# COMBINE-lab/RapMap

Hardware: AMD Instinct MI355X
Metric: Mreads/s (paired 2x100 bp; one unit = one read pair) (higher is better)
Workload: dtype u8/int32/u64 (integer & byte work, no floating point)

## Files before the change

rapmap_amd/csrc/qm_device.h:

```cpp
#pragma once
#include <hip/hip_runtime.h>
#include <stddef.h>

#define QMK_BLOCKS_PER_CU 8
#define QM_SEL_CHUNKS_B 4
#define QMK_DEFAULT_WPS 8
#define QMK_WPS_PH 6
#define QMK_WPS_NIP 8
#define QMK_WPS_PHNIP 6

extern "C" {
hipError_t qmk_build_sainfo(const unsigned int* SA, long long nSA, const unsigned int* offsets, long long T, void* out, hipStream_t st);
hipError_t qmk_build_saext(const unsigned char* text, long long n, const unsigned int* SA, long long nSA, int k, const void* sainfo, void* out, hipStream_t st);
hipError_t qmk_build_saext2(const unsigned char* text, long long n, const unsigned int* SA, long long nSA, int k, const void* sainfo, void* out, hipStream_t st);
size_t qmk_saext2_bytes(void);
hipError_t qmk_build_sanext(const unsigned char* text, long long n, const unsigned int* SA, long long nSA, int k, unsigned int* out, hipStream_t st);
hipError_t qmk_build_slots(const void* recs, long long K, void* slots, unsigned long long cap, int k, hipStream_t st);
hipError_t qmk_build_slots_from_ph(const void* dev_index, long long n, void* slots, unsigned long long cap, unsigned long long* d_bad, hipStream_t st);
hipError_t qmk_build_phrecs(const unsigned int* data, const unsigned char* lens, long long n, const void* dev_index, void* out, hipStream_t st);
hipError_t qmk_build_phfilter(const void* recs, long long n, void* filter, unsigned long long mask, int k, hipStream_t st);
int qmk_map_grid(long long n, int num_cu);
int qmk_map_grid_ex(long long n, int num_cu, int ph_compact);
int qmk_grid_oversub_ph(void);
int qmk_grid_oversub(void);
int qmk_resident_grid(long long n, int num_cu);
hipError_t qmk_launch_reads_ns2(const void* dev_index, const void* read_batch, int collect, int grid, int num_cu, hipStream_t st);
hipError_t qmk_launch_reads_ns3(const void* dev_index, const void* read_batch, int collect, int grid, int num_cu, hipStream_t st);
hipError_t qmk_launch_reads_ns4(const void* dev_index, const void* read_batch, int collect, int grid, int num_cu, hipStream_t st);
hipError_t qmk_launch_reads_ns8(const void* dev_index, const void* read_batch, int collect, int grid, int num_cu, hipStream_t st);
hipError_t qmk_launch_reads_ns32(const void* dev_index, const void* read_batch, int collect, int grid, int num_cu, hipStream_t st);
hipError_t qmk_launch_lean(const void* dev_index, const void* read_batch, int num_cu, hipStream_t st);
hipError_t qmk_launch_lean_nq(const void* dev_index, const void* read_batch, int num_cu, hipStream_t st);
hipError_t qmk_launch_duo(const void* dev_index, const void* read_batch, int num_cu, hipStream_t st);
hipError_t qmk_map_reads(const void* dev_index, const void* read_batch, int ns, int grid, int num_cu, hipStream_t st);
hipError_t qmk_map_reads_ex(const void* dev_index, const void* read_batch, int ns, int collect, int grid, int num_cu, hipStream_t st);
hipError_t qmk_h2m(const void* dev_index, const void* read_batch, int grid, int num_cu, hipStream_t st);
hipError_t qmk_h2m_packw(const void* dev_index, const void* read_batch, const long long* ids, const unsigned long long* nids, long long* todoq, int grid, int num_cu, hipStream_t st);
hipError_t qmk_rebase_offsets(const long long* src, long long* dst, long long n, long long add, hipStream_t st);
hipError_t qmk_h2m_pack(const void* dev_index, const void* read_batch, long long* todoq, int grid, int num_cu, hipStream_t st);
hipError_t qmk_sel_merge(const void* pair_batch, const void* sel_batch, hipStream_t st);
size_t qmk_sel_scratch_bytes(void);
size_t qmk_sel_dyn_struct_bytes(void);
unsigned long long qmk_sel_dyn_bytes(long long n);
void qmk_sel_dyn_bind(void* host_struct, void* dev_base, long long n);
hipError_t qmk_collect_marked(const unsigned int* lcnt, long long nreads, unsigned int mark, long long* q, long long cap, unsigned long long* count, hipStream_t st);
hipError_t qmk_sel_slots(const void* pair_batch, hipStream_t st);
hipError_t qmk_sel_plan(const void* pair_batch, const void* sel_batch, int num_cu, hipStream_t st);
size_t qmk_sel_side_bytes(void);
hipError_t qmk_sel_align_finish(const void* pair_batch, const void* sel_batch, int num_cu, hipStream_t st);
size_t qmk_sel_task_bytes(void);
size_t qmk_sel_gmem_rows_bytes(int num_cu);
hipError_t qmk_sel_compact(const void* pair_batch, const void* tmp, const void* toff, hipStream_t st);
hipError_t qmk_pair_count(const void* pair_batch, hipStream_t st);
hipError_t qmk_pair_write(const void* pair_batch, hipStream_t st);
hipError_t qmk_unpack_reads(const unsigned char* packed, const long long* off, long long n, long long total_chars, unsigned char* seq,
                            const void* exc, long long n_exc, hipStream_t st);
size_t qmk_scan_temp_bytes(long long n);
hipError_t qmk_scan_counts(void* temp, size_t temp_bytes, const unsigned int* cnt, long long* offs, long long n,
                           hipStream_t st);
hipError_t qmk_scan_counts_masked(void* temp, size_t temp_bytes, const unsigned int* cnt, long long* offs, long long n, hipStream_t st);
hipError_t qmk_stage_gather(long long nreads, const unsigned int* ivcnt, const long long* ivoff, const void* iv, const long long* ivcsr, void* iv_out,
                            const unsigned int* lcnt, const long long* loff, const unsigned long long* lists, const long long* lcsr,
                            unsigned long long* words_out, hipStream_t st);
hipError_t qmk_eqc_label_queued(const void* src, long long nq, hipStream_t st);
hipError_t qmk_eqc_reset_probes(unsigned long long* q, long long n, hipStream_t st);
hipError_t qmk_eqc_sum(const unsigned long long* count, const unsigned long long* key, long long cap, unsigned long long* out, hipStream_t st);
int qmk_fld_grid(long long n_units, int num_cu, int max_blocks);
hipError_t qmk_fld_fold(const void* src, const void* acc, int blocks, hipStream_t st);
}
```

rapmap_amd/csrc/qm_host.hip:

```cpp
#include <fcntl.h>
#include <hip/hip_runtime.h>
#include <sys/mman.h>
#include <sys/stat.h>
#include <unistd.h>

#include <atomic>
#include <cmath>
#include <cstdarg>
#include <cstdio>
#include <cstdlib>
#include <cstring>
#include <deque>
#include <string>
#include <vector>
#include <thread>
#include <map>
#include <memory>
#include <mutex>
#include <condition_variable>
#include <functional>

#include "qm_mapper.inl"
#include "qm_lean.inl"
#include "qm_device.h"
// ... 176 lines not shown
  std::vector<std::thread> th; std::mutex mu; std::condition_variable cv, done;
  std::function<void(int)> job; unsigned long gen = 0; int pending = 0, parts = 0; bool stop = false;
  explicit SplitPool(int n) {
    for (int i = 0; i < n; ++i) th.emplace_back([this, i]() {
      unsigned long seen = 0;
      for (;;) {
        std::function<void(int)> j;
        { std::unique_lock<std::mutex> lk(mu); cv.wait(lk, [&] { return stop || (gen != seen && i < parts); }); if (stop) return; seen = gen; j = job; }
        j(i);
        { std::lock_guard<std::mutex> lk(mu); if (--pending == 0) done.notify_all(); }
      }
    });
  }
  void run(int n, std::function<void(int)> f) {
    std::unique_lock<std::mutex> lk(mu);
    job = std::move(f); parts = n; pending = n; ++gen;
    cv.notify_all();
    done.wait(lk, [&] { return pending == 0; });
  }
  ~SplitPool() { { std::lock_guard<std::mutex> lk(mu); stop = true; } cv.notify_all(); for (auto& t : th) t.join(); }
};
struct SplitJoin {
  qm_ctx* owner; int K; std::mutex mu; std::condition_variable cv;
  long long total[8] = {0}, base[9] = {0}; int arrived = 0; bool ready = false; int failed = 0;
  int arrive(int part, long long tot, long long& b, qm_hit*& dst);
  void abort(int rc) { std::lock_guard<std::mutex> lk(mu); if (!failed) failed = rc ? rc : QM_E_STATE; cv.notify_all(); }
  bool stagger = false; int turn = 0;
  int wait_turn(int part) {
    if (!stagger) return QM_OK;
    std::unique_lock<std::mutex> lk(mu);
    cv.wait(lk, [&] { return turn >= part || failed; });
    return failed ? fail(failed, "another part of the batch failed") : QM_OK;
  }
  void pass_turn(int part) { if (!stagger) return; std::lock_guard<std::mutex> lk(mu); if (turn < part + 1) turn = part + 1; cv.notify_all(); }
};

static void begin_call(qm_ctx* c) { c->last.invalidate(); c->stats = CallStats(); }

extern "C" {

const char* qm_last_error(void) { return g_err; }
const char* qm_version(void) { return "qmap_mi355 0.1 (RapMap 0.6.0 quasimap hot path, gfx950)"; }

int qm_opts_default(qm_opts* o) {
  if (!o) return fail(QM_E_ARG, "null opts");
  o->sensitive = 1; o->strict_check = 1; o->max_num_hits = 200; o->no_orphans = 0; o->no_dovetail = 0;
  o->fuzzy = 0; o->max_interval = 1000; o->sel_aln = 0; o->quasi_cov = 0.0;
  o->hard_filter = 0; o->match_score = 2; o->mismatch_penalty = -4; o->gap_open = 4; o->gap_extend = 2; o->dp_bandwidth = 15;
// ... 439 lines not shown

static int check_opts(const qm_opts* o) {
  if (!o) return fail(QM_E_ARG, "null opts");
  if (o->max_num_hits < 0 || o->max_interval < 1) return fail(QM_E_ARG, "bad max_num_hits / max_interval");
  return QM_OK;
}

struct ChunkFeeder {
  int64_t chunk;
  int (*upload)(void* self, int64_t u0, int64_t u1);
  void* self;
};

enum { QM_RUN_FUSED = 0, QM_RUN_COLLECT = 1, QM_RUN_FROM_INTERVALS = 2 };
struct RunReq {
  int mode = QM_RUN_FUSED;
  bool keepIntervals = false;
  bool keepFound = false;
  bool mergeOnly = false;
  bool stageView = false;
  bool longReads = false;
  int shortLen = 0;
  const qm_sa_interval_hit* ivIn = nullptr; const long long* ivInOff = nullptr; const int* lenIn = nullptr; const unsigned char* foundIn = nullptr;
  SplitJoin* join = nullptr; int part = 0;
  bool noDuo = false;
};

static DevIndex dev_index(const qm_ctx* c) {
  const Replica& R = *c->rep;
  DevIndex ix; ix.text = R.text; ix.n = c->ix->n; ix.SA = R.SA; ix.nSA = c->ix->nSA;
  ix.sainfo = (const SaInfo*)R.sainfo.p; ix.slots = (const Bucket*)R.slots.p; ix.hmask = R.cap - 1; ix.ph = R.ph; ix.k = c->ix->k;
  memset(&ix.phv, 0, sizeof(ix.phv)); if (R.ph) ix.phv = R.hPh;
  ix.sanext = c->d_sanext; ix.saext = (const SaExt*)R.saext.p; ix.saext2 = (const SaExt2*)c->d_saext2;
  return ix;
}


static bool ensure_saext2(qm_ctx* c) {
  if (c->d_saext2) return true;
  Replica& R = *c->rep;
  if (!R.saext || c->ix->nSA <= 0 || c->ix->nTxp >= (1LL << QM_EXT2_TID_BITS)) return false;
  std::lock_guard<std::mutex> lk(R.sanextMu);
  if (!R.saext2 && !R.saext2Tried) {
    R.saext2Tried = true;
    size_t freeB = 0, totalB = 0;
    const size_t need = (size_t)c->ix->nSA * qmk_saext2_bytes(), margin = (size_t)8 << 30;
    if (hipMemGetInfo(&freeB, &totalB) != hipSuccess || freeB < need + margin) { (void)hipGetLastError(); return false; }
// ... 349 lines not shown
  return c->d_scanTmp.ensure((int64_t)(stb ? stb : 16));
}

static int run_stage_b(qm_ctx* c, const qm_opts* o, const RunReq& rq, int64_t n, bool paired, const void* d_seq1, const void* d_off1,
                       const void* d_seq2, const void* d_off2, u64* hscal, long long& total) {
  int rc;
  if ((rc = c->d_cnt.ensure(n + 1))) return rc;
  if ((rc = c->d_offs.ensure(n + 1))) return rc;
  if ((rc = ensure_scan_tmp(c, n + 1))) return rc;
  PairBatch P; memset(&P, 0, sizeof(P));
  P.n = n; P.paired = paired ? 1 : 0; P.off1 = (const long long*)d_off1; P.off2 = (const long long*)d_off2;
  P.lcnt = c->d_lcnt; P.loff = c->d_loff; P.lists = c->d_lists; P.cnt = c->d_cnt; P.offs = c->d_offs;
  P.counters = c->d_scal + 1; P.max_num_hits = o->max_num_hits; P.no_orphans = rq.mergeOnly ? 0 : o->no_orphans;
  P.no_dovetail = rq.mergeOnly ? 0 : o->no_dovetail; P.fuzzy = o->fuzzy; P.merge_only = rq.mergeOnly ? 1 : 0;
  if (rq.mergeOnly) {
    if ((rc = c->d_tooMany.ensure(n + 1))) return rc;
    HIPCHK(hipMemsetAsync(c->d_tooMany, 0, (size_t)(n + 1), c->stream));
    P.too_many = c->d_tooMany;
  }
  if (rq.mergeOnly) c->last.tooManyUnits = n;
  HIPCHK(hipMemsetAsync(c->d_cnt + n, 0, sizeof(uint32_t), c->stream));
  if (o->sel_aln) {
    HIPCHK(qmk_sel_slots(&P, c->stream));
    HIPCHK(qmk_scan_counts(c->d_scanTmp, (size_t)c->d_scanTmp.cap, c->d_cnt, c->d_offs, n + 1, c->stream));
    if ((rc = c->d_toff.ensure(n + 1))) return rc;
    HIPCHK(hipMemcpyAsync(c->d_toff, c->d_offs, (size_t)(n + 1) * 8, hipMemcpyDeviceToDevice, c->stream));
    long long slots = 0;
    HIPCHK(hipMemcpyAsync(&slots, c->d_offs + n, sizeof(long long), hipMemcpyDeviceToHost, c->stream));
    const char* cuEnv = getenv("QM_SEL_CHUNK_UNITS");
    const int64_t minChunk = cuEnv && atoll(cuEnv) > 0 ? atoll(cuEnv) : 65536;
    const int K = n >= (int64_t)QM_SEL_CHUNKS_B * minChunk ? QM_SEL_CHUNKS_B : 1;
    long long cu[QM_SEL_CHUNKS_B + 1], cslot[QM_SEL_CHUNKS_B + 1];
    for (int i = 0; i <= K; ++i) { cu[i] = n * i / K; cslot[i] = 0; }
    for (int i = 1; i < K; ++i) HIPCHK(hipMemcpyAsync(&cslot[i], c->d_offs + cu[i], sizeof(long long), hipMemcpyDeviceToHost, c->stream));
    HIPCHK(hipStreamSynchronize(c->stream));
    cslot[K] = slots;
    if ((rc = c->d_tmp.ensure(slots + 1))) return rc;
    if ((rc = c->d_tsc.ensure(2 * slots + 2))) return rc;
    SelBatch A; memset(&A, 0, sizeof(A));
    A.seq1 = (const unsigned char*)d_seq1; A.seq2 = (const unsigned char*)d_seq2; A.text = c->rep->text;
    A.txp_off = c->rep->txpOff; A.txp_len = c->rep->txpLen; A.tmp = c->d_tmp; A.toff = c->d_toff; A.tsc = c->d_tsc;
    A.match = o->match_score; A.mismatch = o->mismatch_penalty; A.gap_open = o->gap_open; A.gap_extend = o->gap_extend;
    A.long_reads = rq.longReads ? 1 : 0;
    if (rq.longReads && !rq.mergeOnly && sel_ksw_ring_slots(o->dp_bandwidth) > 128) {
      if ((rc = c->d_kswRows.ensure((int64_t)qmk_sel_gmem_rows_bytes(c->numCU)))) return rc;
      A.ksw_rows = c->d_kswRows;
    }
// ... 15 lines not shown
      HIPCHK(hipStreamWaitEvent(c->planStream, c->evPlan[QM_SEL_CHUNKS_B], 0));
      SelBatch Ak[QM_SEL_CHUNKS_B];
      static const bool serial = [] { const char* e = getenv("QM_SEL_SERIAL"); return e && atoi(e) != 0; }();
      hipStream_t planStream = K > 1 && !serial ? c->planStream : c->stream;
      for (int i = 0; i < K; ++i) {
        Ak[i] = A; Ak[i].u0 = cu[i]; Ak[i].u1 = cu[i + 1];
        Ak[i].tasks = (SelTask*)(c->d_tasks + (size_t)(2 * cslot[i] + 2 * i) * qmk_sel_task_bytes());
        Ak[i].ntasks = c->d_ntk + i;
        Ak[i].sides = (SelSide*)(c->d_sides + (size_t)(2 * cslot[i] + 2 * i) * qmk_sel_side_bytes());
        Ak[i].nsides = c->d_ntk + QM_SEL_CHUNKS_B + i;
        Ak[i].torder = c->d_torder + (size_t)(2 * cslot[i] + 2 * i);
        if (!noStrip) { Ak[i].torder2 = c->d_torder + (size_t)(2 * slots + 2 * K + 2) + (size_t)(2 * cslot[i] + 2 * i); Ak[i].ntasks2 = c->d_ntk + 2 * QM_SEL_CHUNKS_B + i; }
        HIPCHK(qmk_sel_plan(&P, &Ak[i], c->numCU, planStream));
        if (K > 1) HIPCHK(hipEventRecord(c->evPlan[i], planStream));
      }
      for (int i = 0; i < K; ++i) {
        if (K > 1) HIPCHK(hipStreamWaitEvent(c->stream, c->evPlan[i], 0));
        HIPCHK(qmk_sel_align_finish(&P, &Ak[i], c->numCU, c->stream));
      }
    }
  } else {
    HIPCHK(qmk_pair_count(&P, c->stream));
  }
  HIPCHK(qmk_scan_counts(c->d_scanTmp, (size_t)c->d_scanTmp.cap, c->d_cnt, c->d_offs, n + 1, c->stream));
  total = 0;
  HIPCHK(hipMemcpyAsync(&total, c->d_offs + n, sizeof(long long), hipMemcpyDeviceToHost, c->stream));
  HIPCHK(hipMemcpyAsync(hscal, c->d_scal, QM_SC_WORDS * sizeof(u64), hipMemcpyDeviceToHost, c->stream));
  u64 h[3 * QM_SEL_CHUNKS_B];
  const bool selStats = o->sel_aln && !rq.mergeOnly;
  if (selStats) HIPCHK(hipMemcpyAsync(h, c->d_ntk, sizeof(h), hipMemcpyDeviceToHost, c->stream));
  HIPCHK(hipStreamSynchronize(c->stream));
  if (selStats) {
    for (int i = 0; i < QM_SEL_CHUNKS_B; ++i) { c->stats.kswTasks += (int64_t)h[i]; c->stats.selQuestions += (int64_t)h[QM_SEL_CHUNKS_B + i]; c->stats.stripTasks += (int64_t)h[2 * QM_SEL_CHUNKS_B + i]; }
    static const bool dbg = [] { const char* e = getenv("QM_SEL_DEBUG"); return e && atoi(e) != 0; }();
    if (dbg) fprintf(stderr, "[qm -s] %lld units: %lld alignment questions beyond PERFECT chains, %lld ksw2 alignments, %lld strip alignments\n", (long long)n, (long long)c->stats.selQuestions, (long long)c->stats.kswTasks, (long long)c->stats.stripTasks);
  }
  if (rq.join) {
    long long b = 0; qm_hit* dst = nullptr;
    if ((rc = rq.join->arrive(rq.part, total, b, dst))) return rc;
    P.hits = dst + b;
  } else {
    if ((rc = c->d_hits.ensure((int64_t)total + 1, total / 8))) return rc;
    P.hits = c->d_hits;
  }
  if (o->sel_aln) HIPCHK(qmk_sel_compact(&P, c->d_tmp, c->d_toff, c->stream));
  else HIPCHK(qmk_pair_write(&P, c->stream));
  return QM_OK;
}

static int map_device_impl(qm_ctx* c, const qm_opts* o, int64_t n, const void* d_seq1, const void* d_off1, const void* d_seq2,
                           const void* d_off2, int32_t max_read_len, int64_t* n_hits, qm_counters* counters, ChunkFeeder* feeder,
                           const RunReq& rq = RunReq(), int32_t short_read_len = 0) {
  if (!c || n < 0 || (n > 0 && (!d_seq1 || !d_off1))) return fail(QM_E_ARG, "bad argument");
  int rc = check_opts(o);
  if (rc) return rc;
  if ((d_seq2 == nullptr) != (d_off2 == nullptr)) return fail(QM_E_ARG, "seq2/off2 must both be given or both be null");
  HIPCHK(hipSetDevice(c->device));
  const int pick = (max_read_len > QM_MAX_READ_LEN && short_read_len > 0) ? short_read_len : (max_read_len > QM_MAX_READ_LEN ? QM_MAX_READ_LEN : max_read_len);
  const int ns = pick <= 128 ? 2 : (pick <= 192 ? 3 : (pick <= 256 ? 4 : 8));
  const bool paired = d_seq2 != nullptr;
  u64 hscal[QM_SC_WORDS];
  begin_call(c);
  HIPCHK(hipEventRecord(c->evA, c->stream));
  RunReq r2 = rq;
  r2.keepIntervals = rq.keepIntervals || c->debug != 0;
  r2.longReads = max_read_len > QM_MAX_READ_LEN;
  r2.shortLen = pick;
  if (rq.join && (rc = rq.join->wait_turn(rq.part))) return rc;
  rc = run_stage_a(c, o, r2, n, d_seq1, d_off1, d_seq2, d_off2, ns, feeder, hscal);
  if (rq.join) rq.join->pass_turn(rq.part);
  if (rc) return rc;
  if (r2.stageView) {
    const int64_t nreads = paired ? 2 * n : n;
    if ((rc = c->d_ivcsr.ensure(nreads + 1))) return rc;
    if ((rc = c->d_lcsr.ensure(nreads + 1))) return rc;
    if ((rc = c->h_tot.ensure(2))) return rc;
    if ((rc = ensure_scan_tmp(c, nreads + 1))) return rc;
    if (!r2.keepIntervals) {
      if ((rc = c->d_ivcnt.ensure(nreads + 1))) return rc;
      if ((rc = c->d_ivoff.ensure(nreads + 1))) return rc;
      if ((rc = c->d_iv.ensure(1))) return rc;
      HIPCHK(hipMemsetAsync(c->d_ivcnt, 0, (size_t)(nreads + 1) * sizeof(uint32_t), c->stream));
      HIPCHK(hipMemsetAsync(c->d_ivoff, 0, (size_t)(nreads + 1) * sizeof(long long), c->stream));
    }
    HIPCHK(hipMemsetAsync(c->d_ivcnt + nreads, 0, sizeof(uint32_t), c->stream));
    HIPCHK(hipMemsetAsync(c->d_lcnt + nreads, 0, sizeof(uint32_t), c->stream));
    HIPCHK(qmk_scan_counts(c->d_scanTmp, (size_t)c->d_scanTmp.cap, c->d_ivcnt, c->d_ivcsr, nreads + 1, c->stream));
    HIPCHK(qmk_scan_counts_masked(c->d_scanTmp, (size_t)c->d_scanTmp.cap, c->d_lcnt, c->d_lcsr, nreads + 1, c->stream));
    HIPCHK(hipMemcpyAsync(&c->h_tot[0], c->d_ivcsr + nreads, sizeof(long long), hipMemcpyDeviceToHost, c->stream));
    HIPCHK(hipMemcpyAsync(&c->h_tot[1], c->d_lcsr + nreads, sizeof(long long), hipMemcpyDeviceToHost, c->stream));
    c->last.stReads = nreads;
  }
  long long total = 0;
  if ((rc = run_stage_b(c, o, r2, n, paired, d_seq1, d_off1, d_seq2, d_off2, hscal, total))) return rc;
  HIPCHK(hipEventRecord(c->evB, c->stream));
  HIPCHK(hipStreamSynchronize(c->stream));
  float ms = 0; hipEventElapsedTime(&ms, c->evA, c->evB); c->last.totalMs = ms;
  c->last.units = n; c->last.hits = total; c->last.paired = paired;
  if (r2.stageView) c->last.stUnits = n;
  if (n_hits) *n_hits = total;
  if (counters) *counters = counters_from(hscal);
  return QM_OK;
}

int SplitJoin::arrive(int part, long long tot, long long& b, qm_hit*& dst) {
  std::unique_lock<std::mutex> lk(mu);
  total[part] = tot;
  if (++arrived == K && !failed) {
    for (int i = 0; i < K; ++i) base[i + 1] = base[i] + total[i];
    const int rc = owner->d_hits.ensure((int64_t)base[K] + 1, base[K] / 8);
    if (rc) failed = rc; else ready = true;
    cv.notify_all();
  }
  cv.wait(lk, [&] { return ready || failed; });
  if (failed) return failed == QM_E_NOMEM ? fail(QM_E_NOMEM, "hipMalloc of the result array failed") : fail(failed, "another part of the batch failed");
  b = base[part]; dst = owner->d_hits;
  return QM_OK;
}

static int map_device_split(qm_ctx* c, const qm_opts* o, int K, int64_t n, const void* d_seq1, const void* d_off1, const void* d_seq2,
                            const void* d_off2, int32_t max_read_len, int64_t* n_hits, qm_counters* counters) {
  int rc;
  HIPCHK(hipSetDevice(c->device));
  while ((int)c->helpers.size() < K) {
    qm_ctx* h = nullptr;
    if ((rc = qm_ctx_create_ex(c->ix, c->device, c->flags, &h))) return rc;
    h->isHelper = true; c->helpers.push_back(h);
  }
  if (!c->pool || (int)c->pool->th.size() < K) { delete c->pool; c->pool = new SplitPool(K); }
  if ((rc = c->d_offs.ensure(n + 1))) return rc;
  SplitJoin J; J.owner = c; J.K = K;
  { const char* sg = getenv("QM_SPLIT_STAGGER"); J.stagger = sg ? atoi(sg) != 0 : false; }
  int64_t nh[8] = {0}; qm_counters ctr[8]; int rcs[8] = {0}; char errs[8][256];
  memset(ctr, 0, sizeof(ctr));
  const bool paired = d_seq2 != nullptr;
  static const int firstPct = [] { const char* e = getenv("QM_SPLIT_FIRST"); const int v = e ? atoi(e) : 0; return v > 0 && v < 100 ? v : 0; }();
  static const int duoParts = [] { const char* e = getenv("QM_DUO_PARTS"); return e ? atoi(e) : 0x55; }();
  begin_call(c);
  HIPCHK(hipEventRecord(c->evA, c->stream));
  c->pool->run(K, [&](int i) {
    qm_ctx* h = c->helpers[(size_t)i];
    int64_t u0 = n * i / K, u1 = n * (i + 1) / K;
    if (K == 2 && firstPct > 0) { const int64_t cut = n * firstPct / 100; u0 = i == 0 ? 0 : cut; u1 = i == 0 ? cut : n; }
    RunReq rq; rq.join = &J; rq.part = i;
    rq.noDuo = ((duoParts >> i) & 1) == 0;
    errs[i][0] = 0;
    int r = map_device_impl(h, o, u1 - u0, d_seq1, (const long long*)d_off1 + u0, d_seq2, d_seq2 ? (const long long*)d_off2 + u0 : nullptr,
                            max_read_len, &nh[i], &ctr[i], nullptr, rq);
    if (r == QM_OK) {
      hipError_t e = qmk_rebase_offsets(h->d_offs, c->d_offs + u0, (u1 - u0) + (i == K - 1 ? 1 : 0), J.base[i], h->stream);
      if (e == hipSuccess) e = hipStreamSynchronize(h->stream);
      if (e != hipSuccess) r = fail(QM_E_NOGPU, "rebasing a part's offsets: %s", hipGetErrorString(e));
    }
    if (r != QM_OK) { snprintf(errs[i], sizeof(errs[i]), "%s", g_err); J.abort(r); }
    rcs[i] = r;
  });
  for (int i = 0; i < K; ++i) if (rcs[i]) return fail(rcs[i], "%s", errs[i]);
  HIPCHK(hipEventRecord(c->evB, c->stream));
  HIPCHK(hipEventSynchronize(c->evB));
  float first = 1e30f, last = 0, t = 0;
  for (int i = 0; i < K; ++i) {
    qm_ctx* h = c->helpers[(size_t)i];
    if (hipEventElapsedTime(&t, c->evA, h->ev0) == hipSuccess && t < first) first = t;
    if (hipEventElapsedTime(&t, c->evA, h->ev1) == hipSuccess && t > last) last = t;
  }
  c->last.mapMs = last > first ? last - first : 0;
  float ms = 0; hipEventElapsedTime(&ms, c->evA, c->evB); c->last.totalMs = ms;
  qm_counters sum; memset(&sum, 0, sizeof(sum));
  for (int i = 0; i < K; ++i) {
    sum += ctr[i];
    int64_t u0 = n * i / K;
    if (K == 2 && firstPct > 0) u0 = i == 0 ? 0 : n * firstPct / 100;
    c->stats.add_part(c->helpers[(size_t)i]->stats, paired ? 2 * u0 : u0);
  }
  c->last.units = n; c->last.hits = J.base[K]; c->last.paired = paired;
  if (n_hits) *n_hits = J.base[K];
  if (counters) *counters = sum;
  return QM_OK;
}

int qm_map_device(qm_ctx* c, const qm_opts* o, int64_t n, const void* d_seq1, const void* d_off1, const void* d_seq2,
                  const void* d_off2, int32_t max_read_len, int64_t* n_hits, qm_counters* counters) {
  const char* me = getenv("QM_SPLIT_MIN");
  const int64_t minUnits = me && atoll(me) > 0 ? atoll(me) : ((int64_t)1 << 21);
  if (c && o && !c->isHelper && !c->debug && n >= minUnits && d_seq1 && d_off1 && (d_seq2 == nullptr) == (d_off2 == nullptr) && check_opts(o) == QM_OK) {
    const char* se = getenv("QM_SPLIT");
    int K = se ? atoi(se) : 2;
    if (K > 8) K = 8;
    if (K > 1) return map_device_split(c, o, K, n, d_seq1, d_off1, d_seq2, d_off2, max_read_len, n_hits, counters);
  }
  return map_device_impl(c, o, n, d_seq1, d_off1, d_seq2, d_off2, max_read_len, n_hits, counters, nullptr);
}

static int stage_offsets(qm_ctx* c, int64_t n, const int64_t* off, DevBuf<uint8_t>& d_seq, DevBuf<long long>& d_off, int32_t& maxLen,
                         int32_t& maxShort) {
  for (int64_t i = 0; i < n; ++i) {
    int64_t l = off[i + 1] - off[i];
    if (l < 0) return fail(QM_E_ARG, "offsets not monotone");
    if (l > maxLen) maxLen = (int32_t)(l > 0x7fffffff ? 0x7fffffff : l);
// ... 485 lines not shown
```

rapmap_amd/csrc/qm_kernels.hip:

```cpp
#include <hip/hip_runtime.h>
#include <cstring>
#include <type_traits>
#include <cstdlib>
#include <rocprim/rocprim.hpp>

#include "qm_mapper.inl"
#include "qm_device.h"

namespace qm {

#ifndef QM_H2M_WPS
#define QM_H2M_WPS 4
#endif
template <int F>
__global__ __launch_bounds__(256, QM_H2M_WPS) void qm_h2m_kernel(DevIndex ix, ReadBatch B) {
  __shared__ H2mMem mem[4];
  __shared__ SelLds<(F & QM_F_SEL) != 0> sels[4];
  const int wave = __builtin_amdgcn_readfirstlane((int)(threadIdx.x >> 6));
  const long long gw = (long long)blockIdx.x * 4 + wave;
  qm_tim_begin(wave);
  h2m_wave<F>(ix, B, gw, (long long)gridDim.x * 4, mem[wave], B.gscratch + gw * QM_GSCR_U64, (F & QM_F_SEL) ? B.selscr + gw : nullptr, sels[wave].ptr(),
              ((F & QM_F_SEL) && B.dyn) ? B.dyn + gw : nullptr);
  qm_tim_flush(B.cursor, wave, 32, 8);
}
// ... 611 lines not shown
  if (ns < 0) return qmk_launch_reads_ns8(ixp, bp, 1, grid, num_cu, st);
  if (collect) {
    if (ns == 2) return qmk_launch_reads_ns2(ixp, bp, 1, grid, num_cu, st);
    if (ns == 3) return qmk_launch_reads_ns3(ixp, bp, 1, grid, num_cu, st);
    if (ns > 4) return qmk_launch_reads_ns8(ixp, bp, 1, grid, num_cu, st);
    return qmk_launch_reads_ns4(ixp, bp, 1, grid, num_cu, st);
  }
  if (ns == 2) return qmk_launch_reads_ns2(ixp, bp, 0, grid, num_cu, st);
  if (ns == 3) return qmk_launch_reads_ns3(ixp, bp, 0, grid, num_cu, st);
  if (ns > 4) return qmk_launch_reads_ns8(ixp, bp, 0, grid, num_cu, st);
  return qmk_launch_reads_ns4(ixp, bp, 0, grid, num_cu, st);
}

hipError_t qmk_h2m(const void* ixp, const void* bp, int grid, int num_cu, hipStream_t st) {
  const DevIndex& ix = *(const DevIndex*)ixp;
  const ReadBatch& B = *(const ReadBatch*)bp;
  static int nbSel = 0, nbPlain = 0;
  if (nbSel == 0 && (hipOccupancyMaxActiveBlocksPerMultiprocessor(&nbSel, qm_h2m_kernel<QM_F_SEL>, 256, 0) != hipSuccess || nbSel < 1)) nbSel = 2;
  if (nbPlain == 0 && (hipOccupancyMaxActiveBlocksPerMultiprocessor(&nbPlain, qm_h2m_kernel<0>, 256, 0) != hipSuccess || nbPlain < 1)) nbPlain = 2;
  const int nb = B.selscr ? nbSel : nbPlain;
  const unsigned g = (unsigned)(grid < num_cu * nb ? grid : num_cu * nb);
  if (B.selscr) hipLaunchKernelGGL(qm_h2m_kernel<QM_F_SEL>, dim3(g), dim3(256), 0, st, ix, B);
  else hipLaunchKernelGGL(qm_h2m_kernel<0>, dim3(g), dim3(256), 0, st, ix, B);
  return hipGetLastError();
}
__global__ __launch_bounds__(256) void qm_rebase_offsets_kernel(const long long* src, long long* dst, long long n, long long add) {
  const long long i = (long long)blockIdx.x * 256 + threadIdx.x;
  if (i < n) dst[i] = src[i] + add;
}
hipError_t qmk_rebase_offsets(const long long* src, long long* dst, long long n, long long add, hipStream_t st) {
  if (n <= 0) return hipSuccess;
  hipLaunchKernelGGL(qm_rebase_offsets_kernel, dim3((unsigned)((n + 255) / 256)), dim3(256), 0, st, src, dst, n, add);
  return hipGetLastError();
}
hipError_t qmk_h2m_pack(const void* ixp, const void* bp, long long* todoq, int grid, int num_cu, hipStream_t st) {
  const DevIndex& ix = *(const DevIndex*)ixp;
  const ReadBatch& B = *(const ReadBatch*)bp;
  static int nb = 0;
  if (nb == 0 && (hipOccupancyMaxActiveBlocksPerMultiprocessor(&nb, qm_h2m_pack_kernel, 256, 0) != hipSuccess || nb < 1)) nb = 2;
  const long long cap = (long long)num_cu * nb * qmk_grid_oversub();
  const unsigned g = (unsigned)(grid < cap ? grid : cap);
  hipLaunchKernelGGL(qm_h2m_pack_kernel, dim3(g), dim3(256), 0, st, ix, B, todoq);
  return hipGetLastError();
}
hipError_t qmk_h2m_packw(const void* ixp, const void* bp, const long long* ids, const unsigned long long* nids, long long* todoq, int grid, int num_cu, hipStream_t st) {
  const DevIndex& ix = *(const DevIndex*)ixp;
  const ReadBatch& B = *(const ReadBatch*)bp;
  static int nb = 0;
  if (nb == 0 && (hipOccupancyMaxActiveBlocksPerMultiprocessor(&nb, qm_h2m_packw_kernel, 256, 0) != hipSuccess || nb < 1)) nb = 1;
  const long long cap = (long long)num_cu * nb * qmk_grid_oversub();
  const unsigned g = (unsigned)(grid < cap ? grid : cap);
  hipLaunchKernelGGL(qm_h2m_packw_kernel, dim3(g), dim3(256), 0, st, ix, B, ids, (const u64*)nids, todoq);
  return hipGetLastError();
}
hipError_t qmk_sel_merge(const void* pp, const void* ap, hipStream_t st) {
// ... 85 lines not shown
  const PairBatch& P = *(const PairBatch*)pp;
  if (P.n <= 0) return hipSuccess;
  hipLaunchKernelGGL(qm_pair_write_kernel, dim3((unsigned)((P.n + 255) / 256)), dim3(256), 0, st, P);
  return hipGetLastError();
}

hipError_t qmk_unpack_reads(const unsigned char* packed, const long long* off, long long n, long long total_chars, unsigned char* seq, const void* exc,
                            long long n_exc, hipStream_t st) {
  if (n > 0) {
    const long long threads = n * (long long)QM_UNPACK_TPR;
    hipLaunchKernelGGL(qm_unpack_kernel, dim3((unsigned)((threads + 255) / 256)), dim3(256), 0, st, packed, off, n, seq);
  }
  if (n_exc > 0) hipLaunchKernelGGL(qm_unpack_exc_kernel, dim3((unsigned)((n_exc + 255) / 256)), dim3(256), 0, st, (const qm_pack_exc*)exc, n_exc, seq, (unsigned long long)total_chars);
  return hipGetLastError();
}

size_t qmk_scan_temp_bytes(long long n) {
  size_t bytes = 0;
  auto it = rocprim::make_transform_iterator((const u32*)nullptr, U32ToI64());
  (void)rocprim::exclusive_scan(nullptr, bytes, it, (long long*)nullptr, 0LL, (size_t)n, rocprim::plus<long long>());
  return bytes;
}

hipError_t qmk_scan_counts(void* temp, size_t temp_bytes, const u32* cnt, long long* offs, long long n, hipStream_t st) {
  auto it = rocprim::make_transform_iterator(cnt, U32ToI64());
  return rocprim::exclusive_scan(temp, temp_bytes, it, offs, 0LL, (size_t)n, rocprim::plus<long long>(), st);
}

hipError_t qmk_scan_counts_masked(void* temp, size_t temp_bytes, const u32* cnt, long long* offs, long long n, hipStream_t st) {
  auto it = rocprim::make_transform_iterator(cnt, U32MaskToI64());
  return rocprim::exclusive_scan(temp, temp_bytes, it, offs, 0LL, (size_t)n, rocprim::plus<long long>(), st);
}

hipError_t qmk_stage_gather(long long nreads, const u32* ivcnt, const long long* ivoff, const void* iv, const long long* ivcsr, void* iv_out,
                            const u32* lcnt, const long long* loff, const unsigned long long* lists, const long long* lcsr,
                            unsigned long long* words_out, hipStream_t st) {
  if (nreads <= 0) return hipSuccess;
  hipLaunchKernelGGL(qm_stage_gather_kernel, dim3((unsigned)((nreads * 4 + 255) / 256)), dim3(256), 0, st, nreads, ivcnt, ivoff,
                     (const qm_sa_interval_hit*)iv, ivcsr, (qm_sa_interval_hit*)iv_out, lcnt, loff, (const u64*)lists, lcsr, (u64*)words_out);
  return hipGetLastError();
}

}
```

rapmap_amd/csrc/qm_wave.h:

```cpp
#pragma once
#include <stdint.h>

#ifdef QM_EMU
#define QM_LDS(T) T
#define QM_DEV inline
#define QM_NL 64
#define QM_LANES(l) for (int l = 0; l < 64; ++l)
#define QM_SCALAR(x) ((void)0)
#else
#include <hip/hip_runtime.h>
#define QM_LDS(T) T __attribute__((address_space(3)))
#define QM_DEV __device__ __forceinline__
#define QM_NL 1
#define QM_LANES(l) for (int _qm_once = 0, l = (int)(threadIdx.x & 63); _qm_once < 1; ++_qm_once)
#define QM_SCALAR(x) asm volatile("" : "+s"(x))
#endif

namespace qm {

typedef unsigned long long u64;
typedef unsigned int u32;

template <typename T>
struct LV {
// ... 92 lines not shown
  const short al = (short)a, bl = (short)b, ah = (short)(a >> 16), bh = (short)(b >> 16);
  return (u32)(unsigned short)(al > bl ? al : bl) | ((u32)(unsigned short)(ah > bh ? ah : bh) << 16);
}
QM_DEV u32 pk_max_u(u32 a, u32 b) { const u32 al = a & 0xffffu, bl = b & 0xffffu, ah = a >> 16, bh = b >> 16; return (al > bl ? al : bl) | ((ah > bh ? ah : bh) << 16); }
QM_DEV u32 pk_min_u(u32 a, u32 b) { const u32 al = a & 0xffffu, bl = b & 0xffffu, ah = a >> 16, bh = b >> 16; return (al < bl ? al : bl) | ((ah < bh ? ah : bh) << 16); }
QM_DEV void lane_xor1(const LV<u32>& in, LV<u32>& out) { for (int l = 0; l < 64; ++l) out.v[l] = in.v[l ^ 1]; }
template <typename T> QM_DEV void swap32(const LV<T>& in, LV<T>& out) { for (int l = 0; l < 64; ++l) out.v[l] = in.v[l ^ 32]; }
QM_DEV u32 align_bytes(u32 hi, u32 lo, int shift) { return (u32)((((u64)hi << 32) | lo) >> (8 * shift)); }
struct U4 { u32 x, y, z, w; };
QM_DEV U4 load_16(const void* p) { U4 v; __builtin_memcpy(&v, p, 16); return v; }
QM_DEV long long load_uniform_i64(const long long* p) { return *p; }
QM_DEV void lds_dma_u32(const u32* g, u32* ldsBase, int lane) { ldsBase[lane] = *g; }
QM_DEV void lds_dma_wait() {}
QM_DEV void lds_dma_u128(const void* g, void* ldsBase, int lane) { __builtin_memcpy((unsigned char*)ldsBase + 16 * lane, g, 16); }
QM_DEV void load_32(const void* p, U4& a, U4& b) { a = load_16(p); b = load_16((const unsigned char*)p + 16); }
QM_DEV void load_16x2(const void* p, const void* q, U4& a, U4& b) { a = load_16(p); b = load_16(q); }
QM_DEV void load_8_16(const u64* p8, const u64* p16, u64& a, U4& b) { a = *p8; b = load_16(p16); }
template <int N> QM_DEV void load_8_16xN(const u64* const* B, const int* bit, u64* word, U4* meta) {
  for (int t = 0; t < N; ++t) load_8_16(B[t] + (bit[t] >> 6), B[t] + 6, word[t], meta[t]);
}
QM_DEV void half_ballot(const LV<bool>& b, LV<u32>& out) { const u64 m = ballot(b); for (int l = 0; l < 64; ++l) out.v[l] = (u32)(m >> (l & 32)); }
QM_DEV void half_read(const LV<u32>& x, const LV<int>& idx, LV<u32>& out) { LV<u32> t; for (int l = 0; l < 64; ++l) t.v[l] = x.v[(l & 32) + (idx.v[l] & 31)]; out = t; }
QM_DEV void wave_read(const LV<u32>& x, const LV<int>& idx, LV<u32>& out) { LV<u32> t; for (int l = 0; l < 64; ++l) t.v[l] = x.v[idx.v[l] & 63]; out = t; }
QM_DEV void half_max(LV<int>& x) {
  for (int b = 0; b < 64; b += 32) { int m = x.v[b]; for (int l = b + 1; l < b + 32; ++l) m = x.v[l] > m ? x.v[l] : m; for (int l = b; l < b + 32; ++l) x.v[l] = m; }
}
QM_DEV void load_48(const void* p, U4& a, U4& b, U4& c) { a = load_16(p); b = load_16((const unsigned char*)p + 16); c = load_16((const unsigned char*)p + 32); }
QM_DEV void group_sum_f64(LV<double>& x, int G) {
  static const int pair[4] = {1, 2, 7, 15};
  for (int s = 0; s < (G > 8 ? 4 : 3); ++s) { LV<double> t; for (int l = 0; l < 64; ++l) t.v[l] = x.v[l] + x.v[l ^ pair[s]]; x = t; }
}
QM_DEV double wave_sum_f64(const LV<double>& x) {
  LV<double> t = x;
  group_sum_f64(t, 16);
  return (t.v[0] + t.v[16]) + (t.v[32] + t.v[48]);
}
QM_DEV void quarters_sum_f64(LV<double>& x) {
  for (int s = 16; s <= 32; s <<= 1) { LV<double> t; for (int l = 0; l < 64; ++l) t.v[l] = x.v[l] + x.v[l ^ s]; x = t; }
}
#else
template <int CTRL, int ROWMASK> QM_DEV int dpp_get(int v) { return __builtin_amdgcn_update_dpp(v, v, CTRL, ROWMASK, 0xf, false); }
QM_DEV int wave_max(const LV<int>& x) {
  int v = x.v[0], t;
  t = dpp_get<0x111, 0xf>(v); v = t > v ? t : v;
  t = dpp_get<0x112, 0xf>(v); v = t > v ? t : v;
  t = dpp_get<0x114, 0xf>(v); v = t > v ? t : v;
// ... 108 lines not shown
  u64 x = *p8; v4u y = *(const v4u*)p16;
  asm volatile("" : "+v"(x), "+v"(y));
  a = x; b.x = y.x; b.y = y.y; b.z = y.z; b.w = y.w;
}
template <int N> QM_DEV void load_8_16xN(const u64* const* B, const int* bit, u64* word, U4* meta) {
  typedef u32 v4u __attribute__((ext_vector_type(4)));
  u64 x[N]; v4u y[N];
#pragma unroll
  for (int t = 0; t < N; ++t) { x[t] = B[t][bit[t] >> 6]; y[t] = *(const v4u*)(B[t] + 6); }
#pragma unroll
  for (int t = 0; t < N; ++t) asm volatile("" : "+v"(x[t]), "+v"(y[t]));
#pragma unroll
  for (int t = 0; t < N; ++t) { word[t] = x[t]; meta[t].x = y[t].x; meta[t].y = y[t].y; meta[t].z = y[t].z; meta[t].w = y[t].w; }
}
QM_DEV void half_ballot(const LV<bool>& b, LV<u32>& out) {
  const u64 m = __builtin_amdgcn_ballot_w64(b.v[0]);
  out.v[0] = (threadIdx.x & 32) ? (u32)(m >> 32) : (u32)m;
}
QM_DEV void wave_read(const LV<u32>& x, const LV<int>& idx, LV<u32>& out) {
  out.v[0] = (u32)__builtin_amdgcn_ds_bpermute((int)((u32)(idx.v[0] & 63) << 2), (int)x.v[0]);
}
QM_DEV void half_read(const LV<u32>& x, const LV<int>& idx, LV<u32>& out) {
  out.v[0] = (u32)__builtin_amdgcn_ds_bpermute((int)(((threadIdx.x & 32) + (u32)(idx.v[0] & 31)) << 2), (int)x.v[0]);
}
QM_DEV void half_max(LV<int>& x) {
  int v = x.v[0], t;
  t = dpp_get<0x111, 0xf>(v); v = t > v ? t : v;
  t = dpp_get<0x112, 0xf>(v); v = t > v ? t : v;
  t = dpp_get<0x114, 0xf>(v); v = t > v ? t : v;
  t = dpp_get<0x118, 0xf>(v); v = t > v ? t : v;
  t = dpp_get<0x142, 0xa>(v); v = t > v ? t : v;
  x.v[0] = __builtin_amdgcn_ds_bpermute((int)((threadIdx.x | 31u) << 2), v);
}
QM_DEV void load_48(const void* p, U4& a, U4& b, U4& c) {
  typedef u32 v4u __attribute__((ext_vector_type(4)));
  v4u x = ((const v4u*)p)[0], y = ((const v4u*)p)[1], z = ((const v4u*)p)[2];
  asm volatile("" : "+v"(x), "+v"(y), "+v"(z));
  a.x = x.x; a.y = x.y; a.z = x.z; a.w = x.w; b.x = y.x; b.y = y.y; b.z = y.z; b.w = y.w; c.x = z.x; c.y = z.y; c.z = z.z; c.w = z.w;
}
template <int CTRL> QM_DEV double dpp_get_f64(double v) {
  const u64 b = __builtin_bit_cast(u64, v);
  const u32 lo = (u32)dpp_get<CTRL, 0xf>((int)(u32)b), hi = (u32)dpp_get<CTRL, 0xf>((int)(u32)(b >> 32));
  return __builtin_bit_cast(double, ((u64)hi << 32) | lo);
}
QM_DEV void group_sum_f64(LV<double>& x, int G) {
  double v = x.v[0];
// ... 91 lines not shown
```

Measured before the change: 482.8.

## Overlap split-part hit writes via early placement and direct scan into owner offsets

Replaces the all-parts barrier before writing hits with a staged protocol. Each part waits only for the totals of earlier parts, then scans its counts straight into the owner's offset array, seeded with that base. If the existing result buffer is already big enough, the part writes its hits immediately; otherwise the write is redone after the buffer grows. This removes the separate rebase-offsets kernel and its extra synchronisation, and also flips the default duo-part mask and adds an unused row8_or DPP helper. In exchange, part scans are serialised by prefix order, a host sync is added per part, and a second write pass may be needed when the buffer grows.

```diff
diff --git a/rapmap_amd/csrc/qm_device.h b/rapmap_amd/csrc/qm_device.h
--- a/rapmap_amd/csrc/qm_device.h
+++ b/rapmap_amd/csrc/qm_device.h
@@ -36,7 +36,6 @@
 hipError_t qmk_map_reads_ex(const void* dev_index, const void* read_batch, int ns, int collect, int grid, int num_cu, hipStream_t st);
 hipError_t qmk_h2m(const void* dev_index, const void* read_batch, int grid, int num_cu, hipStream_t st);
 hipError_t qmk_h2m_packw(const void* dev_index, const void* read_batch, const long long* ids, const unsigned long long* nids, long long* todoq, int grid, int num_cu, hipStream_t st);
-hipError_t qmk_rebase_offsets(const long long* src, long long* dst, long long n, long long add, hipStream_t st);
 hipError_t qmk_h2m_pack(const void* dev_index, const void* read_batch, long long* todoq, int grid, int num_cu, hipStream_t st);
 hipError_t qmk_sel_merge(const void* pair_batch, const void* sel_batch, hipStream_t st);
 size_t qmk_sel_scratch_bytes(void);
@@ -56,7 +55,7 @@
 hipError_t qmk_unpack_reads(const unsigned char* packed, const long long* off, long long n, long long total_chars, unsigned char* seq,
                             const void* exc, long long n_exc, hipStream_t st);
 size_t qmk_scan_temp_bytes(long long n);
-hipError_t qmk_scan_counts(void* temp, size_t temp_bytes, const unsigned int* cnt, long long* offs, long long n,
+hipError_t qmk_scan_counts(void* temp, size_t temp_bytes, const unsigned int* cnt, long long* offs, long long n, long long init,
                            hipStream_t st);
 hipError_t qmk_scan_counts_masked(void* temp, size_t temp_bytes, const unsigned int* cnt, long long* offs, long long n, hipStream_t st);
 hipError_t qmk_stage_gather(long long nreads, const unsigned int* ivcnt, const long long* ivoff, const void* iv, const long long* ivcsr, void* iv_out,
diff --git a/rapmap_amd/csrc/qm_host.hip b/rapmap_amd/csrc/qm_host.hip
--- a/rapmap_amd/csrc/qm_host.hip
+++ b/rapmap_amd/csrc/qm_host.hip
@@ -222,8 +222,11 @@
 };
 struct SplitJoin {
   qm_ctx* owner; int K; std::mutex mu; std::condition_variable cv;
-  long long total[8] = {0}, base[9] = {0}; int arrived = 0; bool ready = false; int failed = 0;
-  int arrive(int part, long long tot, long long& b, qm_hit*& dst);
+  long long total[8] = {0}, base[9] = {0}; bool have[8] = {false}; int arrived = 0, inflight = 0; bool needGrow = false, sized = false; int failed = 0;
+  int wait_base(int part, long long& b);
+  int place(int part, long long tot, qm_hit*& dst, bool& early);
+  int settle(int part, bool early, bool& again, qm_hit*& dst);
+  int failure() { return failed == QM_E_NOMEM ? fail(QM_E_NOMEM, "hipMalloc of the result array failed") : fail(failed, "another part of the batch failed"); }
   void abort(int rc) { std::lock_guard<std::mutex> lk(mu); if (!failed) failed = rc ? rc : QM_E_STATE; cv.notify_all(); }
   bool stagger = false; int turn = 0;
   int wait_turn(int part) {
@@ -709,7 +712,7 @@
   bool longReads = false;
   int shortLen = 0;
   const qm_sa_interval_hit* ivIn = nullptr; const long long* ivInOff = nullptr; const int* lenIn = nullptr; const unsigned char* foundIn = nullptr;
-  SplitJoin* join = nullptr; int part = 0;
+  SplitJoin* join = nullptr; int part = 0; int64_t u0 = 0;
   bool noDuo = false;
 };
 
@@ -1105,7 +1108,7 @@
   HIPCHK(hipMemsetAsync(c->d_cnt + n, 0, sizeof(uint32_t), c->stream));
   if (o->sel_aln) {
     HIPCHK(qmk_sel_slots(&P, c->stream));
-    HIPCHK(qmk_scan_counts(c->d_scanTmp, (size_t)c->d_scanTmp.cap, c->d_cnt, c->d_offs, n + 1, c->stream));
+    HIPCHK(qmk_scan_counts(c->d_scanTmp, (size_t)c->d_scanTmp.cap, c->d_cnt, c->d_offs, n + 1, 0, c->stream));
     if ((rc = c->d_toff.ensure(n + 1))) return rc;
     HIPCHK(hipMemcpyAsync(c->d_toff, c->d_offs, (size_t)(n + 1) * 8, hipMemcpyDeviceToDevice, c->stream));
     long long slots = 0;
@@ -1167,9 +1170,14 @@
   } else {
     HIPCHK(qmk_pair_count(&P, c->stream));
   }
-  HIPCHK(qmk_scan_counts(c->d_scanTmp, (size_t)c->d_scanTmp.cap, c->d_cnt, c->d_offs, n + 1, c->stream));
+  long long base = 0; long long* offsOut = c->d_offs;
+  if (rq.join) {
+    if ((rc = rq.join->wait_base(rq.part, base))) return rc;
+    offsOut = rq.join->owner->d_offs + rq.u0;
+  }
+  HIPCHK(qmk_scan_counts(c->d_scanTmp, (size_t)c->d_scanTmp.cap, c->d_cnt, offsOut, n + 1, base, c->stream));
   total = 0;
-  HIPCHK(hipMemcpyAsync(&total, c->d_offs + n, sizeof(long long), hipMemcpyDeviceToHost, c->stream));
+  HIPCHK(hipMemcpyAsync(&total, offsOut + n, sizeof(long long), hipMemcpyDeviceToHost, c->stream));
   HIPCHK(hipMemcpyAsync(hscal, c->d_scal, QM_SC_WORDS * sizeof(u64), hipMemcpyDeviceToHost, c->stream));
   u64 h[3 * QM_SEL_CHUNKS_B];
   const bool selStats = o->sel_aln && !rq.mergeOnly;
@@ -1181,13 +1189,23 @@
     if (dbg) fprintf(stderr, "[qm -s] %lld units: %lld alignment questions beyond PERFECT chains, %lld ksw2 alignments, %lld strip alignments\n", (long long)n, (long long)c->stats.selQuestions, (long long)c->stats.kswTasks, (long long)c->stats.stripTasks);
   }
   if (rq.join) {
-    long long b = 0; qm_hit* dst = nullptr;
-    if ((rc = rq.join->arrive(rq.part, total, b, dst))) return rc;
-    P.hits = dst + b;
-  } else {
-    if ((rc = c->d_hits.ensure((int64_t)total + 1, total / 8))) return rc;
-    P.hits = c->d_hits;
-  }
+    total -= base;
+    qm_hit* dst = nullptr; bool early = false, again = false;
+    if ((rc = rq.join->place(rq.part, total, dst, early))) return rc;
+    P.offs = offsOut;
+    for (int pass = 0; pass < 2; ++pass) {
+      P.hits = dst;
+      if (o->sel_aln) HIPCHK(qmk_sel_compact(&P, c->d_tmp, c->d_toff, c->stream));
+      else HIPCHK(qmk_pair_write(&P, c->stream));
+      if (pass) break;
+      HIPCHK(hipStreamSynchronize(c->stream));
+      if ((rc = rq.join->settle(rq.part, early, again, dst))) return rc;
+      if (!again) break;
+    }
+    return QM_OK;
+  }
+  if ((rc = c->d_hits.ensure((int64_t)total + 1, total / 8))) return rc;
+  P.hits = c->d_hits;
   if (o->sel_aln) HIPCHK(qmk_sel_compact(&P, c->d_tmp, c->d_toff, c->stream));
   else HIPCHK(qmk_pair_write(&P, c->stream));
   return QM_OK;
@@ -1230,7 +1248,7 @@
     }
     HIPCHK(hipMemsetAsync(c->d_ivcnt + nreads, 0, sizeof(uint32_t), c->stream));
     HIPCHK(hipMemsetAsync(c->d_lcnt + nreads, 0, sizeof(uint32_t), c->stream));
-    HIPCHK(qmk_scan_counts(c->d_scanTmp, (size_t)c->d_scanTmp.cap, c->d_ivcnt, c->d_ivcsr, nreads + 1, c->stream));
+    HIPCHK(qmk_scan_counts(c->d_scanTmp, (size_t)c->d_scanTmp.cap, c->d_ivcnt, c->d_ivcsr, nreads + 1, 0, c->stream));
     HIPCHK(qmk_scan_counts_masked(c->d_scanTmp, (size_t)c->d_scanTmp.cap, c->d_lcnt, c->d_lcsr, nreads + 1, c->stream));
     HIPCHK(hipMemcpyAsync(&c->h_tot[0], c->d_ivcsr + nreads, sizeof(long long), hipMemcpyDeviceToHost, c->stream));
     HIPCHK(hipMemcpyAsync(&c->h_tot[1], c->d_lcsr + nreads, sizeof(long long), hipMemcpyDeviceToHost, c->stream));
@@ -1248,18 +1266,46 @@
   return QM_OK;
 }
 
-int SplitJoin::arrive(int part, long long tot, long long& b, qm_hit*& dst) {
+int SplitJoin::wait_base(int part, long long& b) {
   std::unique_lock<std::mutex> lk(mu);
-  total[part] = tot;
-  if (++arrived == K && !failed) {
+  cv.wait(lk, [&] { if (failed) return true; for (int i = 0; i < part; ++i) if (!have[i]) return false; return true; });
+  if (failed) return failure();
+  b = 0;
+  for (int i = 0; i < part; ++i) b += total[i];
+  return QM_OK;
+}
+
+int SplitJoin::place(int part, long long tot, qm_hit*& dst, bool& early) {
+  std::unique_lock<std::mutex> lk(mu);
+  total[part] = tot; have[part] = true; ++arrived;
+  long long b = 0;
+  for (int i = 0; i < part; ++i) b += total[i];
+  cv.notify_all();
+  if (failed) return failure();
+  early = !needGrow && owner->d_hits.p && owner->d_hits.cap >= b + tot + 1;
+  if (early) { ++inflight; dst = owner->d_hits; return QM_OK; }
+  needGrow = true;
+  cv.wait(lk, [&] { return failed || (arrived == K && inflight == 0); });
+  if (failed) return failure();
+  if (!sized) {
     for (int i = 0; i < K; ++i) base[i + 1] = base[i] + total[i];
     const int rc = owner->d_hits.ensure((int64_t)base[K] + 1, base[K] / 8);
-    if (rc) failed = rc; else ready = true;
+    if (rc) { failed = rc; cv.notify_all(); return failure(); }
+    sized = true;
     cv.notify_all();
   }
-  cv.wait(lk, [&] { return ready || failed; });
-  if (failed) return failed == QM_E_NOMEM ? fail(QM_E_NOMEM, "hipMalloc of the result array failed") : fail(failed, "another part of the batch failed");
-  b = base[part]; dst = owner->d_hits;
+  dst = owner->d_hits;
+  return QM_OK;
+}
+
+int SplitJoin::settle(int part, bool early, bool& again, qm_hit*& dst) {
+  std::unique_lock<std::mutex> lk(mu);
+  if (early) { --inflight; cv.notify_all(); }
+  again = false;
+  if (!early) return failed ? failure() : QM_OK;
+  cv.wait(lk, [&] { return failed || (arrived == K && (!needGrow || sized)); });
+  if (failed) return failure();
+  if (needGrow) { again = true; dst = owner->d_hits; }
   return QM_OK;
 }
 
@@ -1280,23 +1326,18 @@
   memset(ctr, 0, sizeof(ctr));
   const bool paired = d_seq2 != nullptr;
   static const int firstPct = [] { const char* e = getenv("QM_SPLIT_FIRST"); const int v = e ? atoi(e) : 0; return v > 0 && v < 100 ? v : 0; }();
-  static const int duoParts = [] { const char* e = getenv("QM_DUO_PARTS"); return e ? atoi(e) : 0x55; }();
+  auto first_unit = [&](int i) { return (K == 2 && firstPct > 0) ? (i == 0 ? (int64_t)0 : (i == 1 ? n * firstPct / 100 : n)) : n * i / K; };
+  static const int duoParts = [] { const char* e = getenv("QM_DUO_PARTS"); return e ? atoi(e) : 0xAA; }();
   begin_call(c);
   HIPCHK(hipEventRecord(c->evA, c->stream));
   c->pool->run(K, [&](int i) {
     qm_ctx* h = c->helpers[(size_t)i];
-    int64_t u0 = n * i / K, u1 = n * (i + 1) / K;
-    if (K == 2 && firstPct > 0) { const int64_t cut = n * firstPct / 100; u0 = i == 0 ? 0 : cut; u1 = i == 0 ? cut : n; }
-    RunReq rq; rq.join = &J; rq.part = i;
+    const int64_t u0 = first_unit(i), u1 = first_unit(i + 1);
+    RunReq rq; rq.join = &J; rq.part = i; rq.u0 = u0;
     rq.noDuo = ((duoParts >> i) & 1) == 0;
     errs[i][0] = 0;
     int r = map_device_impl(h, o, u1 - u0, d_seq1, (const long long*)d_off1 + u0, d_seq2, d_seq2 ? (const long long*)d_off2 + u0 : nullptr,
                             max_read_len, &nh[i], &ctr[i], nullptr, rq);
-    if (r == QM_OK) {
-      hipError_t e = qmk_rebase_offsets(h->d_offs, c->d_offs + u0, (u1 - u0) + (i == K - 1 ? 1 : 0), J.base[i], h->stream);
-      if (e == hipSuccess) e = hipStreamSynchronize(h->stream);
-      if (e != hipSuccess) r = fail(QM_E_NOGPU, "rebasing a part's offsets: %s", hipGetErrorString(e));
-    }
     if (r != QM_OK) { snprintf(errs[i], sizeof(errs[i]), "%s", g_err); J.abort(r); }
     rcs[i] = r;
   });
@@ -1312,14 +1353,15 @@
   c->last.mapMs = last > first ? last - first : 0;
   float ms = 0; hipEventElapsedTime(&ms, c->evA, c->evB); c->last.totalMs = ms;
   qm_counters sum; memset(&sum, 0, sizeof(sum));
+  long long hits = 0;
   for (int i = 0; i < K; ++i) {
     sum += ctr[i];
-    int64_t u0 = n * i / K;
-    if (K == 2 && firstPct > 0) u0 = i == 0 ? 0 : n * firstPct / 100;
+    const int64_t u0 = first_unit(i);
     c->stats.add_part(c->helpers[(size_t)i]->stats, paired ? 2 * u0 : u0);
-  }
-  c->last.units = n; c->last.hits = J.base[K]; c->last.paired = paired;
-  if (n_hits) *n_hits = J.base[K];
+    hits += J.total[i];
+  }
+  c->last.units = n; c->last.hits = hits; c->last.paired = paired;
+  if (n_hits) *n_hits = hits;
   if (counters) *counters = sum;
   return QM_OK;
 }
diff --git a/rapmap_amd/csrc/qm_kernels.hip b/rapmap_amd/csrc/qm_kernels.hip
--- a/rapmap_amd/csrc/qm_kernels.hip
+++ b/rapmap_amd/csrc/qm_kernels.hip
@@ -657,15 +657,6 @@
   const unsigned g = (unsigned)(grid < num_cu * nb ? grid : num_cu * nb);
   if (B.selscr) hipLaunchKernelGGL(qm_h2m_kernel<QM_F_SEL>, dim3(g), dim3(256), 0, st, ix, B);
   else hipLaunchKernelGGL(qm_h2m_kernel<0>, dim3(g), dim3(256), 0, st, ix, B);
-  return hipGetLastError();
-}
-__global__ __launch_bounds__(256) void qm_rebase_offsets_kernel(const long long* src, long long* dst, long long n, long long add) {
-  const long long i = (long long)blockIdx.x * 256 + threadIdx.x;
-  if (i < n) dst[i] = src[i] + add;
-}
-hipError_t qmk_rebase_offsets(const long long* src, long long* dst, long long n, long long add, hipStream_t st) {
-  if (n <= 0) return hipSuccess;
-  hipLaunchKernelGGL(qm_rebase_offsets_kernel, dim3((unsigned)((n + 255) / 256)), dim3(256), 0, st, src, dst, n, add);
   return hipGetLastError();
 }
 hipError_t qmk_h2m_pack(const void* ixp, const void* bp, long long* todoq, int grid, int num_cu, hipStream_t st) {
@@ -797,9 +788,9 @@
   return bytes;
 }
 
-hipError_t qmk_scan_counts(void* temp, size_t temp_bytes, const u32* cnt, long long* offs, long long n, hipStream_t st) {
+hipError_t qmk_scan_counts(void* temp, size_t temp_bytes, const u32* cnt, long long* offs, long long n, long long init, hipStream_t st) {
   auto it = rocprim::make_transform_iterator(cnt, U32ToI64());
-  return rocprim::exclusive_scan(temp, temp_bytes, it, offs, 0LL, (size_t)n, rocprim::plus<long long>(), st);
+  return rocprim::exclusive_scan(temp, temp_bytes, it, offs, init, (size_t)n, rocprim::plus<long long>(), st);
 }
 
 hipError_t qmk_scan_counts_masked(void* temp, size_t temp_bytes, const u32* cnt, long long* offs, long long n, hipStream_t st) {
diff --git a/rapmap_amd/csrc/qm_wave.h b/rapmap_amd/csrc/qm_wave.h
--- a/rapmap_amd/csrc/qm_wave.h
+++ b/rapmap_amd/csrc/qm_wave.h
@@ -138,6 +138,9 @@
 QM_DEV void half_ballot(const LV<bool>& b, LV<u32>& out) { const u64 m = ballot(b); for (int l = 0; l < 64; ++l) out.v[l] = (u32)(m >> (l & 32)); }
 QM_DEV void half_read(const LV<u32>& x, const LV<int>& idx, LV<u32>& out) { LV<u32> t; for (int l = 0; l < 64; ++l) t.v[l] = x.v[(l & 32) + (idx.v[l] & 31)]; out = t; }
 QM_DEV void wave_read(const LV<u32>& x, const LV<int>& idx, LV<u32>& out) { LV<u32> t; for (int l = 0; l < 64; ++l) t.v[l] = x.v[idx.v[l] & 63]; out = t; }
+QM_DEV void row8_or(LV<u32>& x) {
+  for (int b = 0; b < 64; b += 8) { u32 m = 0; for (int l = b; l < b + 8; ++l) m |= x.v[l]; for (int l = b; l < b + 8; ++l) x.v[l] = m; }
+}
 QM_DEV void half_max(LV<int>& x) {
   for (int b = 0; b < 64; b += 32) { int m = x.v[b]; for (int l = b + 1; l < b + 32; ++l) m = x.v[l] > m ? x.v[l] : m; for (int l = b; l < b + 32; ++l) x.v[l] = m; }
 }
@@ -292,6 +295,13 @@
 }
 QM_DEV void half_read(const LV<u32>& x, const LV<int>& idx, LV<u32>& out) {
   out.v[0] = (u32)__builtin_amdgcn_ds_bpermute((int)(((threadIdx.x & 32) + (u32)(idx.v[0] & 31)) << 2), (int)x.v[0]);
+}
+QM_DEV void row8_or(LV<u32>& x) {
+  int v = (int)x.v[0];
+  v |= __builtin_amdgcn_update_dpp(0, v, 0xB1, 0xf, 0xf, true);
+  v |= __builtin_amdgcn_update_dpp(0, v, 0x4E, 0xf, 0xf, true);
+  v |= __builtin_amdgcn_update_dpp(0, v, 0x141, 0xf, 0xf, true);
+  x.v[0] = (u32)v;
 }
 QM_DEV void half_max(LV<int>& x) {
   int v = x.v[0], t;
```

Result: faster. 494.1 (median of 6 runs) (+2.3%).
